# Nextomics/NextPolish2

Hardware: AMD Instinct MI355X
Metric: polished reference Mbp/s (whole node) at 30x HiFi + k21/k31; FASTA identical to oracle (higher is better)
Workload: dtype u8

## Files before the change

### nextpolish2_amd/csrc/np2_host.cpp

```cpp
#include "../../include/np2.h"
#include "np2_common.hpp"
#include "np2_kernels.hpp"
#include "np2_ctx.hpp"
#include "np2_phase_host.hpp"

#include <algorithm>
#include <atomic>
#include <thread>
#include <chrono>
#include <cstdio>
#include <cstdlib>
#include <cstring>
#include <map>
#include <mutex>
#include <stdexcept>
#include <string>
#include <unordered_map>
#include <unordered_set>
#include <future>
#include <functional>
#include <vector>

using namespace np2;

// ... 166 lines not shown
    std::vector<uint32_t> cur_lo(R), cur_up(R);
    for (uint32_t v = 0; v < R; ++v) {
        cur_lo[v] = vd.off_own[v], cur_up[v] = vd.off_own[v] + n_lo[v];
        vd.off_own[v + 1] = cur_up[v] + n_up[v];
    }
    vd.edges_own.resize(vd.off_own[R]);
    for (uint64_t i = 0; i < np; ++i) {
        uint32_t a, b;
        if (!listed(i, a, b)) continue;
        const int32_t same = (int32_t)(cn[i] & 0xFFFFu), neg = (int32_t)(cn[i] >> 16);
        const float w = (float)(neg >= 3 ? -neg : same - neg);
        vd.edges_own[cur_lo[b]++] = phase::Graph::Edge(a, w);
        vd.edges_own[cur_up[a]++] = phase::Graph::Edge(b, w);
    }
    vd.off = vd.off_own.data(), vd.edges = vd.edges_own.data(), vd.n_nokey = nokey;
    return true;
}

void vote_collect(np2_ctx *cx, np2_contig *c, PassCounts &pc, bool asref, bool use_all, int pass, uint32_t own_lo,
                  uint32_t own_hi, VoteData &vd, bool wide = false, uint64_t key_add = 0) {
    hipStream_t s = cx->stream;
    const uint32_t R = c->R, n_reg = pc.n_reg;
    RegionTables rt = region_tables(cx, n_reg);
    uint32_t NE = 0, NU = 0;
    vd = VoteData();
    vd.R = R;
    {
        EventTimer t(cx, "vote_phase");
        cx->reg_lable.ensure(n_reg + 2);
        cx->grp.ensure((size_t)pc.NC_cap + 2);
        cx->ecount.ensure(n_reg + 2);
        cx->eoff.ensure(std::max<size_t>(n_reg + 2, (size_t)c->L + 2));
        const size_t RP = ((size_t)R + 63) & ~(size_t)63;
        const size_t band_words = (size_t)R * EDGE_BAND;
        const size_t b_v = RP * 10, b_off = (((size_t)R + 2) * 4 + 15) & ~(size_t)15;
        uint8_t *vbuf;
        uint32_t *row_off;
        if (wide) {
            cx->votebuf.ensure(b_v);
            cx->band_off.ensure((size_t)R + 2);
            vbuf = cx->votebuf.p, row_off = cx->band_off.p;
        } else {
            cx->votepack.ensure(b_v + b_off + band_words * 2 * sizeof(phase::Graph::Edge) + 64);
            vbuf = cx->votepack.p, row_off = (uint32_t *)(cx->votepack.p + b_v);
        }
        uint32_t *v_first = (uint32_t *)vbuf;
        int32_t *v_refw = (int32_t *)(vbuf + RP * 4);
        uint8_t *v_seen = vbuf + RP * 8, *v_bad = vbuf + RP * 9;
        op_fill(cx, v_first, 0xFF, RP * 4);
        op_fill(cx, v_refw, 0, RP * 6);
        launch_vote_phase(s, rt, asref, use_all, cx->lq_start.p, own_lo, own_hi, cx->reg_lable.p, cx->grp.p, cx->ecount.p,
                          v_refw, v_seen, v_bad, v_first, cx->scal.p + S_ERR);
        exclusive_total_n(cx, cx->ecount.p, cx->eoff.p, n_reg);
        launch_vote_counts(s, v_first, v_bad, R, cx->scal.p + S_M1);
        cx->band.ensure(band_words + 4);
        cx->band_n.ensure((size_t)R + 2);
        op_fill(cx, cx->scal.p + S_M3, 0, 4);
        launch_edges_row(s, rt, cx->grp.p, cx->ecount.p, cx->pj.p, cx->pcount.p, cx->alive.p, R, cx->band.p, cx->band_n.p,
                         cx->scal.p + S_M3);
        if (wide) {
            exclusive_total_n(cx, cx->band_n.p, row_off, R);
            cx->ekey.ensure(band_words + 2);
            cx->eval.ensure(band_words + 2);
            launch_band_emit(s, cx->band.p, R, row_off, cx->ekey.p, cx->eval.p, cx->scal.p + S_NRAW, key_add);
        } else {
            cx->row_cnt.ensure((size_t)R + 2);
            launch_vote_rows_count(s, cx->band.p, cx->band_n.p, v_bad, use_all, R, cx->row_cnt.p, cx->scal.p + S_NOKEY);
            exclusive_total_n(cx, cx->row_cnt.p, row_off, R);
            launch_vote_rows_emit(s, cx->band.p, cx->band_n.p, v_bad, use_all, v_first, R, row_off, cx->votepack.p + b_v + b_off,
                                  cx->scal.p + S_NRAW, cx->scal.p + S_NOKEY);
        }
    }
    const size_t RP = ((size_t)R + 63) & ~(size_t)63;
    const size_t b_v = RP * 10, b_off = (((size_t)R + 2) * 4 + 15) & ~(size_t)15;
    auto per_read = [&](const uint8_t *vb) {
        vd.first_key.assign((const uint32_t *)vb, (const uint32_t *)vb + R);
        vd.ref_w.assign((const int32_t *)(vb + RP * 4), (const int32_t *)(vb + RP * 4) + R);
        vd.ref_seen.assign(vb + RP * 8, vb + RP * 8 + R);
        vd.bad.assign(vb + RP * 9, vb + RP * 9 + R);
    };
    bool far = false, have_per_read = false;
    {
        std::vector<uint32_t> sc;
        uint8_t *pin = nullptr;
        const size_t EB = sizeof(phase::Graph::Edge);
        static_assert(sizeof(phase::Graph::Edge) == 8 && alignof(phase::Graph::Edge) <= 8, "an edge is {u32 neighbour, f32 weight}");
        const uint32_t likely = (uint32_t)std::min<size_t>((size_t)R * EDGE_BAND * 2, std::max<size_t>((size_t)R * 128, 1u << 15));
        if (wide) {
            sc = fetch_scal(cx, cx->scal.p + S_M0, cx->eoff.p + n_reg);
        } else {
            pin = (uint8_t *)cx->pin_d2h.ensure(b_v + b_off + (size_t)likely * EB + 64);
            const uint32_t seq = ++cx->mbox_seq;
            launch_post(cx->stream, cx->scal.p, S_COUNT, cx->mbox_dev, seq, cx->scal.p + S_M0, cx->eoff.p + n_reg, nullptr, nullptr,
                        nullptr, nullptr, nullptr, nullptr, nullptr, nullptr);
            op_d2h(cx, pin, cx->votepack.p, b_v + b_off);
            launch_copy_counted(cx->stream, (uint32_t *)(pin + b_v + b_off), (const uint32_t *)(cx->votepack.p + b_v + b_off),
                                (const uint32_t *)(cx->votepack.p + b_v) + R, likely * (uint32_t)(EB / 4), (uint32_t)(EB / 4));
            op_sync(cx);
            if (__atomic_load_n(&cx->mbox_host[0], __ATOMIC_ACQUIRE) != seq)
                throw Np2Error(NP2_E_DEVICE, "mailbox not posted after a synchronisation");
            sc.assign(cx->mbox_host + 1, cx->mbox_host + 1 + S_COUNT);
        }
        check_region_err(cx, sc[S_ERR]);
        pc.resolve(sc);
        NE = sc[S_M0];
        if (!cx->trace && sc[S_M1] == 0 && sc[S_M2] == 0) {
            if (NE) throw Np2Error(NP2_E_DEVICE, "internal: pair edges without voting reads");
            return;
        }
        NU = sc[S_NRAW];
        far = sc[S_M3] != 0 || cx->hooks.edge_sort;
        if (!wide) cx->timing.host.push_back({far ? "vote_sort" : "vote_rows", 1.0f});
        if (!wide) {
            per_read(pin);
            have_per_read = true;
            vd.d_bad = cx->votepack.p + RP * 9;
            if (!far) {
                if (NU > likely) {
                    pin = (uint8_t *)cx->pin_d2h.ensure(b_v + b_off + (size_t)NU * EB + 64);
                    op_d2h(cx, pin, cx->votepack.p, b_v + b_off + (size_t)NU * EB);
// ... 2123 lines not shown
```

### nextpolish2_amd/csrc/np2_kernels.hpp

```cpp
#pragma once
#include <cstddef>
#include <cstdint>
#include <hip/hip_runtime.h>
#include "../../include/np2.h"
#include "np2_lookback.hpp"
#include "np2_launch.hpp"

namespace np2 {

static constexpr uint32_t TILE_SHIFT = 10;
static constexpr uint32_t TILE = 1u << TILE_SHIFT;
static constexpr uint32_t TILE_CAP = 4096;

static constexpr uint32_t DENSE_COLS = 4096;
struct ChunkDesc {
    uint64_t nib_off;
    uint64_t ckbase;
    uint32_t read, ts;
    uint32_t c0, ncols;
    uint32_t first_chunk;
    uint32_t aln_t_e, nck;
    uint32_t pad0;
    uint32_t pad[4];
};
// ... 208 lines not shown
static constexpr uint32_t PF_CAP_BIG = 3584;
static constexpr uint32_t PF_COV_MAX = 8192;
static constexpr uint32_t PF_REDO = 1u;
static constexpr uint32_t PF_NEED_BIG = 2u;
struct PfTile {
    const uint64_t *keys;
    const uint32_t *vals;
    const uint32_t *tile_n, *tile_scan;
    const uint16_t *pidx;
    const uint8_t *alive;
    const np2_read_t *reads;
    const uint32_t *tile_rd_off, *tile_rd;
    const uint8_t *refnib;
    uint16_t *slots;
    uint32_t *tile_cnt, *tile_lq;
    long long *tile_gain;
    uint32_t *flags, *n_bad, *bad_list, *n_bad2, *bad_list2;
    long long *end_rel;
    unsigned long long *gain_total;
    unsigned long long *prof;
    uint32_t L, n_tiles, bucket_cap;
    uint32_t cap_lim, cap_lim_big, halo_lim, cov_max;
    uint32_t big_enabled;
};
uint64_t pf_slot_entries(uint32_t n_tiles, uint64_t T);
void launch_pf_tile(hipStream_t s, const PfTile &a);
void launch_pf_compact(hipStream_t s, uint32_t n_tiles, const uint16_t *slots, const uint32_t *tile_scan, const uint32_t *tile_cnt,
                       const uint32_t *tile_coff, const uint32_t *tile_lqoff, uint32_t *cns_pos, uint8_t *cns_base,
                       uint8_t *cns_cls, uint8_t *lq_nothead, uint32_t *lq_list, uint32_t lq_cap, uint32_t *err, uint32_t *flags,
                       uint32_t *flags_out, uint32_t *n_bad, uint32_t *n_bad2);

struct RegionTables {
    const uint32_t *cand_off;
    const uint32_t *order;
    uint16_t *kscore;
    const uint32_t *seq_off;
    const uint8_t *seq;
    uint32_t n_reg;
};
struct RechPtrs {
    const void *groups;
    const uint32_t *job_off;
    const uint32_t *rech;
    const uint32_t *cand_off;
    const uint32_t *keep_list;
    const uint32_t *seq_off;
    const uint8_t *seq;
    const uint8_t *cns_base;
    uint32_t n_groups;
};
void launch_vote_phase(hipStream_t s, const RegionTables &rt, bool asref, bool use_all, const uint32_t *lq_start,
                       uint32_t own_lo, uint32_t own_hi, uint8_t *reg_lable, uint8_t *grp, uint32_t *ecount, int32_t *ref_w,
                       uint8_t *ref_seen, uint8_t *bad, uint32_t *first_reg, uint32_t *err);
void launch_vote_counts(hipStream_t s, const uint32_t *first_reg, const uint8_t *bad, uint32_t R, uint32_t *out);
void launch_edges_write(hipStream_t s, const RegionTables &rt, const uint8_t *reg_lable, const uint8_t *grp,
                        const uint32_t *ecount, const uint32_t *eoff, uint64_t *ekey, uint32_t *eval);
static constexpr uint32_t EDGE_BAND = 256;
void launch_edges_row(hipStream_t s, const RegionTables &rt, const uint8_t *grp, const uint32_t *ecount, const uint32_t *pj,
                      const uint32_t *pcount, const uint8_t *alive, uint32_t R, uint32_t *band, uint32_t *row_n, uint32_t *ovf);
void launch_band_emit(hipStream_t s, const uint32_t *band, uint32_t R, const uint32_t *row_off, uint64_t *ukey, uint32_t *uw,
                      uint32_t *n_out, uint64_t key_add = 0);
void launch_vote_rows_count(hipStream_t s, const uint32_t *band, const uint32_t *row_n, const uint8_t *bad, bool use_all, uint32_t R,
                            uint32_t *cnt, uint32_t *nokey);
void launch_vote_rows_emit(hipStream_t s, const uint32_t *band, const uint32_t *row_n, const uint8_t *bad, bool use_all,
                           const uint32_t *first_reg, uint32_t R, const uint32_t *off, void *edges, uint32_t *n_out, uint32_t *nokey);
void launch_edge_reduce(hipStream_t s, const uint64_t *ekey, const uint32_t *eval, uint32_t n, uint32_t *flag, uint32_t *wout);
void launch_edge_compact(hipStream_t s, const uint64_t *ekey, const uint32_t *flag, const uint32_t *idx, const uint32_t *wout,
                         uint32_t n, uint64_t *ukey, uint32_t *uw, uint32_t *n_out);
void launch_seed(hipStream_t s, const RegionTables &rt, int32_t max_indel_len, uint8_t *reg_lable, uint32_t *seed_cand,
                 uint32_t *keep_n, uint32_t *keep_list, uint16_t *keep_ks, uint32_t *err, uint32_t *rl_list = nullptr,
                 uint32_t *rl_cnt = nullptr, uint32_t rl_cap = 0);
uint32_t region_lb_blocks(uint32_t n_reg);
void launch_splice_find(hipStream_t s, const uint32_t *cns_pos, const uint32_t *M_p, const uint32_t *lq_start,
                        const uint32_t *lq_end, const uint8_t *reg_lable, uint8_t lable, uint32_t n_reg, uint32_t *idx_s,
                        uint32_t *idx_e, uint32_t *stuck);
void launch_splice_plan(hipStream_t s, const Lookback &lb, const uint8_t *reg_lable, uint8_t lable, uint32_t n_reg,
                        const uint32_t *stuck, const uint32_t *idx_s, const uint32_t *idx_e, const uint32_t *seed_cand,
                        const uint32_t *seq_off, uint32_t *ap_g, uint32_t *ap_s, uint32_t *ap_e, int32_t *ap_delta,
                        int32_t *ap_shift_incl, uint32_t *n_ap, const uint32_t *M_in, uint32_t *M_out, uint32_t out_cap , uint32_t *err);
void launch_splice_write(hipStream_t s, const uint32_t *in_pos, const uint8_t *in_base, const uint32_t *M_p, uint32_t M_cap,
                         const uint32_t *ap_g, const uint32_t *ap_s, const uint32_t *ap_e, const int32_t *ap_delta,
                         const int32_t *ap_shift_incl, const uint32_t *n_ap, uint32_t max_ap, const uint32_t *lq_start,
                         const uint32_t *seed_cand, const uint32_t *seq_off, const uint8_t *seq, uint32_t *out_pos,
                         uint8_t *out_base);
void launch_shard_bounds(hipStream_t s, const uint32_t *cns_pos, const uint32_t *M_p, const uint32_t *t, uint32_t *out);
void launch_rech_list(hipStream_t s, const Lookback &lb, const uint8_t *reg_lable, uint32_t n_reg, uint32_t *rech,
                      uint32_t *n_rech, unsigned long long *blob_bound, uint32_t *err);
void launch_rech_groups(hipStream_t s, const Lookback &lb, const uint32_t *rech, const uint32_t *n_rech_p, uint32_t max_rech,
                        const uint32_t *cns_pos, const uint32_t *M_p, const uint32_t *lq_start, const uint32_t *lq_end,
                        const uint32_t *keep_n, uint32_t ksize, const uint32_t *reg_maxlen, void *tmp_groups,
                        uint32_t *head_jobs, void *groups, uint32_t *job_off, uint32_t *n_groups, uint32_t *n_jobs,
                        unsigned long long *blob_bound, uint32_t *err);
size_t rech_group_bytes();
void launch_rech_job_len(hipStream_t s, const RechPtrs &p, uint32_t n_jobs, uint32_t *len);
void launch_rech_job_build(hipStream_t s, const RechPtrs &p, uint32_t n_jobs, const uint32_t *soff32, uint64_t *soff64,
                           uint8_t *blob);
void launch_rech_apply(hipStream_t s, const RechPtrs &p, const uint16_t *score, uint16_t *keep_ks);
void launch_rech_select(hipStream_t s, const uint32_t *rech, const uint32_t *n_rech_p, uint32_t max_rech,
                        const uint32_t *cand_off, const uint32_t *keep_n, const uint32_t *keep_list, const uint16_t *keep_ks,
                        const uint32_t *order, bool first_yak, uint8_t *reg_lable, uint32_t *seed_cand);
void launch_rech_relabel(hipStream_t s, uint8_t *reg_lable, uint32_t n_reg);
static constexpr uint32_t RL_CAP_LIST = 1024;
static constexpr uint32_t RL_CAP_JOBS = 2048;
static constexpr uint32_t RL_CAP_BLOB = 1u << 20;
static constexpr uint32_t RL_NREG_MAX = 400000;
enum : uint32_t { RL_N = 0, RL_NGROUPS, RL_NJOBS, RL_OFF, RL_STATE_WORDS };
struct RechList {
    const uint32_t *list_in;
    uint32_t *cnt_in;
    uint32_t *list_out, *cnt_out;
    uint32_t *st;
    uint32_t *rech;
    uint32_t *pos_lo, *pos_ub;
    void *groups, *tmp_groups;
    uint32_t *job_off, *blob_off, *glen;
    uint2 *job_ol;
// ... 43 lines not shown
```

### nextpolish2_amd/csrc/np2_regions.hip

```cpp
#include "np2_common.hpp"
#include "np2_kernels.hpp"
#include "np2_blockscan.hpp"
#include "np2_lookback.hpp"

namespace np2 {

static constexpr uint8_t LB_TEMP = 0x01, LB_SUCC = 0x80, LB_HETE = 0x40, LB_RECH = 0x20;

__device__ __forceinline__ uint32_t min_support(uint32_t n) { return n >= 9 ? 3u : (n >= 6 ? 2u : 1u); }

struct SubWave {
    uint32_t base;
    bool half;
    __device__ __forceinline__ uint64_t ballot(bool p) const {
        const uint64_t b = __ballot(p);
        return half ? (b >> base) & 0xFFFFFFFFull : b;
    }
    template <class T> __device__ __forceinline__ T shfl(T v, uint32_t j) const { return __shfl(v, (int)(base + j)); }
};

struct WaveStats {
    uint64_t eqmask;
    uint32_t stat;
    uint32_t c;
// ... 191 lines not shown
                    if (wgt < 0 && !use_all) bad[order] = 1;
                }
                const uint64_t V = ref_valid ? (valid & ~1ull) : valid;
                const uint32_t m = __builtin_popcountll(V);
                if (m >= 2 && owned) {
                    ne = m * (m - 1) / 2;
                    if ((V >> lane) & 1ull) atomicMin(&first_reg[order], g);
                }
            }
        }
        if (lane == 0) {
            reg_lable[g] = lable;
            ecount[g] = ne;
        }
    }
}

__device__ __forceinline__ void k_edges_write(const uint32_t np2_bid, const uint32_t np2_nb, RegionTables rt, const uint8_t *__restrict__ reg_lable,
                                                     const uint8_t *__restrict__ grp,
                                                     const uint32_t *__restrict__ ecount,
                                                     const uint32_t *__restrict__ eoff, uint64_t *__restrict__ ekey,
                                                     uint32_t *__restrict__ eval) {
    const uint32_t lane = threadIdx.x & 63;
    const uint32_t g = (uint32_t)__builtin_amdgcn_readfirstlane((int)((np2_bid * blockDim.x + threadIdx.x) >> 6));
    if (g >= rt.n_reg || ecount[g] == 0) return;
    const uint32_t c0 = rt.cand_off[g], n = rt.cand_off[g + 1] - c0;
    uint32_t order = 0xFFFFFFFFu, gi = 0;
    bool v = false;
    if (lane < n) {
        order = rt.order[c0 + lane];
        gi = grp[c0 + lane];
        v = rt.kscore[c0 + lane] > 0;
    }
    uint64_t V = __ballot(v);
    if ((V & 1ull) && __shfl(order, 0) == 0) V &= ~1ull;
    const bool mine = (V >> lane) & 1ull;
    const uint32_t cnt = mine ? __builtin_popcountll(lane == 63 ? 0ull : (V >> (lane + 1))) : 0u;
    uint32_t inc = cnt;
    for (int o = 1; o < 64; o <<= 1) {
        const uint32_t t = __shfl_up(inc, o);
        if (lane >= (uint32_t)o) inc += t;
    }
    uint32_t o = eoff[g] + inc - cnt;
    for (uint32_t j = 1; j < n; ++j) {
        const uint32_t oj = __shfl(order, j), gj = __shfl(gi, j);
        if (mine && j > lane && ((V >> j) & 1ull)) {
            ekey[o] = ((uint64_t)order << 32) | oj;
            eval[o] = (gj == gi) ? 1u : 0xFFFFFFFFu;
            ++o;
        }
    }
}

__device__ __forceinline__ void k_edges_row(const uint32_t np2_bid0, const uint32_t np2_nb, RegionTables rt, const uint8_t *__restrict__ grp,
                                            const uint32_t *__restrict__ ecount, const uint32_t *__restrict__ pj,
                                            const uint32_t *__restrict__ pcount, const uint8_t *__restrict__ alive, uint32_t R,
                                            uint32_t *__restrict__ band, uint32_t *__restrict__ row_n, uint32_t *__restrict__ ovf) {
    const uint32_t np2_bid = xcd_order(np2_bid0, np2_nb);
    __shared__ uint32_t s_row[4][EDGE_BAND];
    const uint32_t lane = threadIdx.x & 63, wv = (uint32_t)__builtin_amdgcn_readfirstlane((int)(threadIdx.x >> 6));
    const uint32_t a = np2_bid * 4 + wv;
    if (a >= R) return;
    uint32_t *row = s_row[wv];
    *reinterpret_cast<uint4 *>(row + lane * 4) = make_uint4(0, 0, 0, 0);
    uint32_t far = 0;
    const uint32_t n_span = (a != 0 && alive[a]) ? pcount[a] : 0u;
    const uint32_t j0 = n_span ? pj[a] : 0u;
    const uint32_t hl = lane & 31, hsel = lane >> 5;
    for (uint32_t base = 0; base < n_span; base += 64) {
        const uint32_t gl = j0 + base + lane;
        const bool in = base + lane < n_span && gl < rt.n_reg;
        const uint32_t c0l = in ? rt.cand_off[gl] : 0u, c1l = in ? rt.cand_off[gl + 1] : 0u;
        uint64_t het = __ballot(in && ecount[gl] != 0);
        while (het) {
            const uint32_t i0 = (uint32_t)__builtin_ctzll(het);
            het &= het - 1;
            const uint32_t c0a = (uint32_t)__builtin_amdgcn_readlane((int)c0l, (int)i0);
            const uint32_t na = (uint32_t)__builtin_amdgcn_readlane((int)c1l, (int)i0) - c0a;
            uint32_t c0b = 0, nb = 0;
            bool two = false;
            if (het && na <= 32) {
                const uint32_t i1 = (uint32_t)__builtin_ctzll(het);
                c0b = (uint32_t)__builtin_amdgcn_readlane((int)c0l, (int)i1);
                nb = (uint32_t)__builtin_amdgcn_readlane((int)c1l, (int)i1) - c0b;
                two = nb <= 32;
                if (two) het &= het - 1;
            }
            const uint32_t li = two ? hl : lane;
            const uint32_t c0 = (two && hsel) ? c0b : c0a, n = (two && hsel) ? nb : na;
            uint32_t order = 0xFFFFFFFFu, gi = 0;
            bool v = false;
            if (li < n) {
                order = rt.order[c0 + li];
                gi = grp[c0 + li];
                v = rt.kscore[c0 + li] > 0;
            }
            uint64_t V = __ballot(v);
            if ((V & 1ull) && __shfl(order, 0) == 0) V &= ~1ull;
            if (two && ((V >> 32) & 1ull) && __shfl(order, 32) == 0) V &= ~(1ull << 32);
            const uint64_t me = __ballot(order == a) & V;
            const uint64_t half_mask = two ? (hsel ? 0xFFFFFFFF00000000ull : 0x00000000FFFFFFFFull) : ~0ull;
            const uint64_t mine = me & half_mask;
            if (!me) continue;
            const uint32_t ga = __shfl(gi, mine ? (int)__builtin_ctzll(mine) : 0);
            if (mine && ((V >> lane) & 1ull) && order > a) {
                const uint32_t d = order - a - 1;
                if (d < EDGE_BAND)
                    atomicAdd(&row[d], gi == ga ? 1u : 0x10000u);
                else
                    ++far;
            }
        }
    }
    const uint4 w = *reinterpret_cast<const uint4 *>(row + lane * 4);
    uint32_t c = (w.x != 0) + (w.y != 0) + (w.z != 0) + (w.w != 0);
    for (int o = 32; o > 0; o >>= 1) c += __shfl_xor(c, o);
    if (c) *reinterpret_cast<uint4 *>(band + (uint64_t)a * EDGE_BAND + lane * 4) = w;
    if (lane == 0) row_n[a] = c;
    for (int o = 32; o > 0; o >>= 1) far += __shfl_xor(far, o);
    if (far && lane == 0) atomicAdd(ovf, far);
}
__device__ __forceinline__ void k_band_emit(const uint32_t np2_bid, const uint32_t np2_nb, const uint32_t *__restrict__ band, uint32_t R,
                                            const uint32_t *__restrict__ row_off, uint64_t *__restrict__ ukey,
                                            uint32_t *__restrict__ ucnt, uint32_t *__restrict__ n_out, uint64_t key_add) {
    const uint32_t lane = threadIdx.x & 63;
    const uint32_t a = (uint32_t)__builtin_amdgcn_readfirstlane((int)((np2_bid * blockDim.x + threadIdx.x) >> 6));
    if (a >= R) return;
    if (a == R - 1 && lane == 0) *n_out = row_off[R];
    if (row_off[a + 1] == row_off[a]) return;
    const uint4 w = *reinterpret_cast<const uint4 *>(band + (uint64_t)a * EDGE_BAND + lane * 4);
    const uint32_t v[4] = {w.x, w.y, w.z, w.w};
    const uint32_t c = (w.x != 0) + (w.y != 0) + (w.z != 0) + (w.w != 0);
    uint32_t inc = c;
    for (int o = 1; o < 64; o <<= 1) {
        const uint32_t t = __shfl_up(inc, o);
        if (lane >= (uint32_t)o) inc += t;
    }
    uint32_t o = row_off[a] + inc - c;
#pragma unroll
    for (uint32_t k = 0; k < 4; ++k)
        if (v[k]) {
            ukey[o] = (((uint64_t)a << 32) | (a + 1 + lane * 4 + k)) + key_add;
            ucnt[o] = v[k];
            ++o;
        }
}

__device__ __forceinline__ uint32_t vote_row_above(const uint32_t *__restrict__ band, const uint8_t *__restrict__ bad, uint32_t use_all,
                                                   uint32_t R, uint32_t v, uint32_t d) {
    const uint32_t b = v + 1 + d;
    if (b >= R) return 0;
    const uint32_t w = band[(uint64_t)v * EDGE_BAND + d];
    return (w != 0 && (use_all || !bad[b])) ? w : 0u;
}
__device__ __forceinline__ uint32_t vote_row_below(const uint32_t *__restrict__ band, const uint32_t *__restrict__ row_n,
                                                   const uint8_t *__restrict__ bad, uint32_t use_all, uint32_t v, int64_t a) {
    if (a < 1 || a >= (int64_t)v || v - (uint32_t)a > EDGE_BAND) return 0;
    if (row_n[a] == 0 || (!use_all && bad[a])) return 0;
    return band[(uint64_t)a * EDGE_BAND + (v - (uint32_t)a - 1)];
}
__device__ __forceinline__ float vote_weight(uint32_t w) {
    const int32_t same = (int32_t)(w & 0xFFFFu), neg = (int32_t)(w >> 16);
    return (float)(neg >= 3 ? -neg : same - neg);
}
__device__ __forceinline__ void k_vote_rows_count(const uint32_t np2_bid, const uint32_t np2_nb, const uint32_t *__restrict__ band,
                                                  const uint32_t *__restrict__ row_n, const uint8_t *__restrict__ bad, uint32_t use_all,
                                                  uint32_t R, uint32_t *__restrict__ cnt, uint32_t *__restrict__ nokey) {
    const uint32_t lane = threadIdx.x & 63;
    const uint32_t v = (uint32_t)__builtin_amdgcn_readfirstlane((int)((np2_bid * blockDim.x + threadIdx.x) >> 6));
    if (v >= R) return;
    if (v == 0 && lane == 0) *nokey = 0;
    uint32_t c = 0;
    if (v != 0 && (use_all || !bad[v])) {
        const bool own = row_n[v] != 0;
#pragma unroll
        for (uint32_t k = 0; k < EDGE_BAND / 64; ++k) {
            const uint32_t d = k * 64 + lane;
            if (own) c += vote_row_above(band, bad, use_all, R, v, d) != 0;
            c += vote_row_below(band, row_n, bad, use_all, v, (int64_t)v - 1 - d) != 0;
        }
    }
    for (int o = 32; o > 0; o >>= 1) c += __shfl_xor(c, o);
    if (lane == 0) cnt[v] = c;
}
__device__ __forceinline__ void k_vote_rows_emit(const uint32_t np2_bid, const uint32_t np2_nb, const uint32_t *__restrict__ band,
                                                 const uint32_t *__restrict__ row_n, const uint8_t *__restrict__ bad, uint32_t use_all,
                                                 const uint32_t *__restrict__ first_reg, uint32_t R, const uint32_t *__restrict__ off,
                                                 uint2 *__restrict__ edges, uint32_t *__restrict__ n_out, uint32_t *__restrict__ nokey) {
    const uint32_t lane = threadIdx.x & 63;
    const uint32_t v = (uint32_t)__builtin_amdgcn_readfirstlane((int)((np2_bid * blockDim.x + threadIdx.x) >> 6));
    if (v >= R) return;
    if (v == R - 1 && lane == 0) *n_out = off[R];
    if (v == 0) return;
    const bool own = row_n[v] != 0, live = use_all || !bad[v];
    const uint64_t lt = (1ull << lane) - 1;
    uint32_t o = off[v];
    const uint32_t end = off[v + 1];
    if (live && end != o) {
#pragma unroll
        for (uint32_t k = 0; k < EDGE_BAND / 64; ++k) {
            const int64_t a = (int64_t)v - EDGE_BAND + k * 64 + lane;
            const uint32_t w = vote_row_below(band, row_n, bad, use_all, v, a);
            const uint64_t m = __ballot(w != 0);
            const uint32_t at = o + (uint32_t)__popcll(m & lt);
            if (w != 0 && at < end) edges[at] = make_uint2((uint32_t)a, __float_as_uint(vote_weight(w)));
            o += (uint32_t)__popcll(m);
        }
    }
    if (!own) return;
    const bool v_key = first_reg[v] != 0xFFFFFFFFu;
    uint32_t nk = 0;
#pragma unroll
    for (uint32_t k = 0; k < EDGE_BAND / 64; ++k) {
        const uint32_t d = k * 64 + lane, b = v + 1 + d;
        if (b < R && band[(uint64_t)v * EDGE_BAND + d] != 0 && !(v_key && first_reg[b] != 0xFFFFFFFFu)) ++nk;
        const uint32_t w = live ? vote_row_above(band, bad, use_all, R, v, d) : 0u;
        const uint64_t m = __ballot(w != 0);
        const uint32_t at = o + (uint32_t)__popcll(m & lt);
        if (w != 0 && at < end) edges[at] = make_uint2(b, __float_as_uint(vote_weight(w)));
        o += (uint32_t)__popcll(m);
    }
    for (int x = 32; x > 0; x >>= 1) nk += __shfl_xor(nk, x);
    if (nk && lane == 0) atomicAdd(nokey, nk);
}

__device__ __forceinline__ void k_edge_reduce(const uint32_t np2_bid, const uint32_t np2_nb, const uint64_t *__restrict__ ekey, const uint32_t *__restrict__ eval, uint32_t n,
                              uint32_t *__restrict__ flag, uint32_t *__restrict__ wout) {
    uint32_t i = np2_bid * blockDim.x + threadIdx.x;
    if (i >= n) return;
    const uint64_t k = ekey[i];
    if (i > 0 && ekey[i - 1] == k) {
        flag[i] = 0;
        return;
    }
    int32_t sum = 0, neg = 0;
    for (uint32_t j = i; j < n && ekey[j] == k; ++j) {
// ... 801 lines not shown
    }
    __syncthreads();
    const uint32_t stuck = s_stuck;
    uint32_t flag[RL_ITEMS], fsum = 0;
    int32_t delta[RL_ITEMS], dsum_t = 0;
#pragma unroll
    for (uint32_t k = 0; k < RL_ITEMS; ++k) {
        flag[k] = (tid * RL_ITEMS + k < n && g[k] + 1 > stuck) ? 1u : 0u;
        delta[k] = 0;
        if (flag[k]) {
            const uint32_t c = seed_cand[g[k]];
            delta[k] = (int32_t)(seq_off[c + 1] - seq_off[c]) - (int32_t)(e[k] - s[k]);
        }
        fsum += flag[k], dsum_t += delta[k];
    }
    uint32_t cnt, dsum;
    uint32_t lo = block_excl_scan<OpAdd, 4>(fsum, sh, cnt);
    uint32_t ld = block_excl_scan<OpAdd, 4>((uint32_t)dsum_t, sh, dsum);
#pragma unroll
    for (uint32_t k = 0; k < RL_ITEMS; ++k) {
        if (flag[k]) {
            ap_g[lo] = g[k];
            ap_s[lo] = s[k];
            ap_e[lo] = e[k];
            ap_delta[lo] = delta[k];
            ap_shift_incl[lo] = (int32_t)ld + delta[k];
        }
        lo += flag[k];
        ld += (uint32_t)delta[k];
    }
    if (tid == 0) splice_plan_total(M, dsum, cnt, out_cap, n_ap, M_out, err);
    uint32_t keep[RL_ITEMS], ksum = 0;
#pragma unroll
    for (uint32_t k = 0; k < RL_ITEMS; ++k) {
        keep[k] = 0;
        if (tid * RL_ITEMS + k < n) {
            const uint8_t l = rech_relabel(reg_lable[g[k]]);
            reg_lable[g[k]] = l;
            keep[k] = (l & LB_RECH) ? 1u : 0u;
        }
        ksum += keep[k];
    }
    uint32_t n_keep;
    uint32_t lk = block_excl_scan<OpAdd, 4>(ksum, sh, n_keep);
#pragma unroll
    for (uint32_t k = 0; k < RL_ITEMS; ++k) {
        if (keep[k]) a.list_out[lk] = g[k];
        lk += keep[k];
    }
    if (tid == 0) *a.cnt_in = 0, *a.cnt_out = last_round ? 0u : n_keep;
}

__device__ __forceinline__ void k_vote_counts(const uint32_t np2_bid, const uint32_t np2_nb, const uint32_t *__restrict__ first_reg, const uint8_t *__restrict__ bad,
                                                      uint32_t R, uint32_t *__restrict__ out) {
    __shared__ uint32_t sk[16], sb[16];
    uint32_t nk = 0, nb = 0;
    for (uint32_t r = threadIdx.x; r < R; r += 1024) {
        nk += first_reg[r] != 0xFFFFFFFFu ? 1u : 0u;
        nb += bad[r] ? 1u : 0u;
    }
    for (int o = 32; o > 0; o >>= 1) {
        nk += __shfl_xor(nk, o);
        nb += __shfl_xor(nb, o);
    }
    if ((threadIdx.x & 63) == 0) {
        sk[threadIdx.x >> 6] = nk;
        sb[threadIdx.x >> 6] = nb;
    }
    __syncthreads();
    if (threadIdx.x == 0) {
        uint32_t a = 0, b = 0;
        for (int i = 0; i < 16; ++i) {
            a += sk[i];
            b += sb[i];
        }
        out[0] = a;
        out[1] = b;
    }
}

static inline dim3 g1(uint64_t n, uint32_t bs = 256) { return dim3((unsigned)((n + bs - 1) / bs)); }

void launch_vote_phase(hipStream_t s, const RegionTables &rt, bool asref, bool use_all, const uint32_t *lq_start,
                       uint32_t own_lo, uint32_t own_hi, uint8_t *reg_lable, uint8_t *grp, uint32_t *ecount, int32_t *ref_w,
                       uint8_t *ref_seen, uint8_t *bad, uint32_t *first_reg, uint32_t *err) {
    if (rt.n_reg)
        NP2_LAUNCH(k_vote_phase, g1((uint64_t)((rt.n_reg + 1) / 2) * 64), 256, s, rt, asref ? 1u : 0u, use_all ? 1u : 0u, lq_start, own_lo, own_hi, reg_lable, grp, ecount, ref_w, ref_seen, bad, first_reg, err);
}
void launch_vote_counts(hipStream_t s, const uint32_t *first_reg, const uint8_t *bad, uint32_t R, uint32_t *out) {
    NP2_LAUNCH(k_vote_counts, dim3(1), 1024, s, first_reg, bad, R, out);
}
void launch_edges_write(hipStream_t s, const RegionTables &rt, const uint8_t *reg_lable, const uint8_t *grp,
                        const uint32_t *ecount, const uint32_t *eoff, uint64_t *ekey, uint32_t *eval) {
    if (rt.n_reg)
        NP2_LAUNCH(k_edges_write, g1((uint64_t)rt.n_reg * 64), 256, s, rt, reg_lable, grp, ecount, eoff, ekey, eval);
}
void launch_edges_row(hipStream_t s, const RegionTables &rt, const uint8_t *grp, const uint32_t *ecount, const uint32_t *pj,
                      const uint32_t *pcount, const uint8_t *alive, uint32_t R, uint32_t *band, uint32_t *row_n, uint32_t *ovf) {
    if (R) NP2_LAUNCH(k_edges_row, g1((uint64_t)R * 64), 256, s, rt, grp, ecount, pj, pcount, alive, R, band, row_n, ovf);
}
void launch_vote_rows_count(hipStream_t s, const uint32_t *band, const uint32_t *row_n, const uint8_t *bad, bool use_all, uint32_t R,
                            uint32_t *cnt, uint32_t *nokey) {
    if (R) NP2_LAUNCH(k_vote_rows_count, g1((uint64_t)R * 64), 256, s, band, row_n, bad, use_all ? 1u : 0u, R, cnt, nokey);
}
void launch_vote_rows_emit(hipStream_t s, const uint32_t *band, const uint32_t *row_n, const uint8_t *bad, bool use_all,
                           const uint32_t *first_reg, uint32_t R, const uint32_t *off, void *edges, uint32_t *n_out, uint32_t *nokey) {
    if (R) NP2_LAUNCH(k_vote_rows_emit, g1((uint64_t)R * 64), 256, s, band, row_n, bad, use_all ? 1u : 0u, first_reg, R, off, (uint2 *)edges, n_out, nokey);
}
void launch_band_emit(hipStream_t s, const uint32_t *band, uint32_t R, const uint32_t *row_off, uint64_t *ukey, uint32_t *uw,
                      uint32_t *n_out, uint64_t key_add) {
    if (R) NP2_LAUNCH(k_band_emit, g1((uint64_t)R * 64), 256, s, band, R, row_off, ukey, uw, n_out, key_add);
}
void launch_edge_reduce(hipStream_t s, const uint64_t *ekey, const uint32_t *eval, uint32_t n, uint32_t *flag,
                        uint32_t *wout) {
    if (n) NP2_LAUNCH(k_edge_reduce, g1(n), 256, s, ekey, eval, n, flag, wout);
}
void launch_edge_compact(hipStream_t s, const uint64_t *ekey, const uint32_t *flag, const uint32_t *idx,
                         const uint32_t *wout, uint32_t n, uint64_t *ukey, uint32_t *uw, uint32_t *n_out) {
    if (n) NP2_LAUNCH(k_edge_compact, g1(n), 256, s, ekey, flag, idx, wout, n, ukey, uw, n_out);
}
void launch_seed(hipStream_t s, const RegionTables &rt, int32_t max_indel_len, uint8_t *reg_lable, uint32_t *seed_cand,
                 uint32_t *keep_n, uint32_t *keep_list, uint16_t *keep_ks, uint32_t *err, uint32_t *rl_list, uint32_t *rl_cnt,
                 uint32_t rl_cap) {
    if (rt.n_reg)
        NP2_LAUNCH(k_seed, g1((uint64_t)((rt.n_reg + 1) / 2) * 64), 256, s, rt, max_indel_len, reg_lable, seed_cand, keep_n, keep_list, keep_ks, err, rl_list, rl_cnt, rl_cap);
}
uint32_t region_lb_blocks(uint32_t n_reg) { return (n_reg + 256 * LB_REG_ITEMS - 1) / (256 * LB_REG_ITEMS); }
void launch_splice_find(hipStream_t s, const uint32_t *cns_pos, const uint32_t *M_p, const uint32_t *lq_start,
                        const uint32_t *lq_end, const uint8_t *reg_lable, uint8_t lable, uint32_t n_reg,
                        uint32_t *idx_s, uint32_t *idx_e, uint32_t *stuck) {
    NP2_LAUNCH(k_splice_find, g1(n_reg), 256, s, cns_pos, M_p, lq_start, lq_end, reg_lable, lable, n_reg, idx_s, idx_e, stuck);
}
void launch_splice_plan(hipStream_t s, const Lookback &lb, const uint8_t *reg_lable, uint8_t lable, uint32_t n_reg,
                        const uint32_t *stuck, const uint32_t *idx_s, const uint32_t *idx_e, const uint32_t *seed_cand,
                        const uint32_t *seq_off, uint32_t *ap_g, uint32_t *ap_s, uint32_t *ap_e, int32_t *ap_delta,
                        int32_t *ap_shift_incl, uint32_t *n_ap, const uint32_t *M_in, uint32_t *M_out, uint32_t out_cap, uint32_t *err) {
    const uint32_t nb = region_lb_blocks(n_reg);
    NP2_LAUNCH(k_splice_plan, dim3(nb), 256, s, lb, nb, reg_lable, lable, n_reg, stuck, idx_s, idx_e, seed_cand, seq_off, ap_g, ap_s, ap_e, ap_delta, ap_shift_incl, n_ap, M_in, M_out, out_cap, err);
}
void launch_splice_write(hipStream_t s, const uint32_t *in_pos, const uint8_t *in_base, const uint32_t *M_p, uint32_t M_cap,
                         const uint32_t *ap_g, const uint32_t *ap_s, const uint32_t *ap_e, const int32_t *ap_delta,
                         const int32_t *ap_shift_incl, const uint32_t *n_ap, uint32_t max_ap, const uint32_t *lq_start,
                         const uint32_t *seed_cand, const uint32_t *seq_off, const uint8_t *seq, uint32_t *out_pos,
                         uint8_t *out_base) {
    NP2_LAUNCH(k_splice_bases, dim3((M_cap + SPLICE_SPAN - 1) / SPLICE_SPAN), 256, s, in_pos, in_base, M_p, ap_s, ap_e, ap_shift_incl, n_ap, out_pos, out_base);
    if (max_ap)
        NP2_LAUNCH(k_splice_seeds, g1((uint64_t)max_ap * 8, 256), 256, s, ap_g, ap_s, ap_delta, ap_shift_incl, n_ap, lq_start, seed_cand, seq_off, seq, out_pos, out_base);
}
void launch_shard_bounds(hipStream_t s, const uint32_t *cns_pos, const uint32_t *M_p, const uint32_t *t, uint32_t *out) {
    NP2_LAUNCH(k_shard_bounds, dim3(1), 64, s, cns_pos, M_p, t[0], t[1], t[2], t[3], t[4], t[5], out);
}
void launch_rech_list(hipStream_t s, const Lookback &lb, const uint8_t *reg_lable, uint32_t n_reg, uint32_t *rech,
                      uint32_t *n_rech, unsigned long long *blob_bound, uint32_t *err) {
    const uint32_t nb = region_lb_blocks(n_reg);
    NP2_LAUNCH(k_rech_list, dim3(nb), 256, s, lb, nb, reg_lable, n_reg, rech, n_rech, blob_bound, err);
}
// ... 53 lines not shown
```

Baseline: 4500.

## Fuse vote row counting into edge row kernel and unroll candidate walk

Removes the separate vote_rows_count kernel: the edge-row kernel now counts per-row edges with atomics on both endpoints while it still holds the band row in registers. The overflow and nokey zeroing moves into vote_counts, which also clears the cnt array, dropping a fill op. The candidate walk is unrolled four ways to batch loads, and the row popcount uses ballots. This saves launches and a band re-read, but adds global atomics on cnt and changes how the count is derived, which risks output divergence.

```diff
diff --git a/nextpolish2_amd/csrc/np2_host.cpp b/nextpolish2_amd/csrc/np2_host.cpp
--- a/nextpolish2_amd/csrc/np2_host.cpp
+++ b/nextpolish2_amd/csrc/np2_host.cpp
@@ -242,20 +242,19 @@
         launch_vote_phase(s, rt, asref, use_all, cx->lq_start.p, own_lo, own_hi, cx->reg_lable.p, cx->grp.p, cx->ecount.p,
                           v_refw, v_seen, v_bad, v_first, cx->scal.p + S_ERR);
         exclusive_total_n(cx, cx->ecount.p, cx->eoff.p, n_reg);
-        launch_vote_counts(s, v_first, v_bad, R, cx->scal.p + S_M1);
+        if (!wide) cx->row_cnt.ensure((size_t)R + 2);
+        launch_vote_counts(s, v_first, v_bad, R, cx->scal.p + S_M1, cx->scal.p + S_M3, wide ? nullptr : cx->row_cnt.p,
+                           wide ? nullptr : cx->scal.p + S_NOKEY);
         cx->band.ensure(band_words + 4);
         cx->band_n.ensure((size_t)R + 2);
-        op_fill(cx, cx->scal.p + S_M3, 0, 4);
         launch_edges_row(s, rt, cx->grp.p, cx->ecount.p, cx->pj.p, cx->pcount.p, cx->alive.p, R, cx->band.p, cx->band_n.p,
-                         cx->scal.p + S_M3);
+                         cx->scal.p + S_M3, v_bad, use_all, wide ? nullptr : cx->row_cnt.p);
         if (wide) {
             exclusive_total_n(cx, cx->band_n.p, row_off, R);
             cx->ekey.ensure(band_words + 2);
             cx->eval.ensure(band_words + 2);
             launch_band_emit(s, cx->band.p, R, row_off, cx->ekey.p, cx->eval.p, cx->scal.p + S_NRAW, key_add);
         } else {
-            cx->row_cnt.ensure((size_t)R + 2);
-            launch_vote_rows_count(s, cx->band.p, cx->band_n.p, v_bad, use_all, R, cx->row_cnt.p, cx->scal.p + S_NOKEY);
             exclusive_total_n(cx, cx->row_cnt.p, row_off, R);
             launch_vote_rows_emit(s, cx->band.p, cx->band_n.p, v_bad, use_all, v_first, R, row_off, cx->votepack.p + b_v + b_off,
                                   cx->scal.p + S_NRAW, cx->scal.p + S_NOKEY);
diff --git a/nextpolish2_amd/csrc/np2_kernels.hpp b/nextpolish2_amd/csrc/np2_kernels.hpp
--- a/nextpolish2_amd/csrc/np2_kernels.hpp
+++ b/nextpolish2_amd/csrc/np2_kernels.hpp
@@ -284,16 +284,16 @@
 void launch_vote_phase(hipStream_t s, const RegionTables &rt, bool asref, bool use_all, const uint32_t *lq_start,
                        uint32_t own_lo, uint32_t own_hi, uint8_t *reg_lable, uint8_t *grp, uint32_t *ecount, int32_t *ref_w,
                        uint8_t *ref_seen, uint8_t *bad, uint32_t *first_reg, uint32_t *err);
-void launch_vote_counts(hipStream_t s, const uint32_t *first_reg, const uint8_t *bad, uint32_t R, uint32_t *out);
+void launch_vote_counts(hipStream_t s, const uint32_t *first_reg, const uint8_t *bad, uint32_t R, uint32_t *out, uint32_t *ovf,
+                        uint32_t *cnt, uint32_t *nokey);
 void launch_edges_write(hipStream_t s, const RegionTables &rt, const uint8_t *reg_lable, const uint8_t *grp,
                         const uint32_t *ecount, const uint32_t *eoff, uint64_t *ekey, uint32_t *eval);
 static constexpr uint32_t EDGE_BAND = 256;
 void launch_edges_row(hipStream_t s, const RegionTables &rt, const uint8_t *grp, const uint32_t *ecount, const uint32_t *pj,
-                      const uint32_t *pcount, const uint8_t *alive, uint32_t R, uint32_t *band, uint32_t *row_n, uint32_t *ovf);
+                      const uint32_t *pcount, const uint8_t *alive, uint32_t R, uint32_t *band, uint32_t *row_n, uint32_t *ovf,
+                      const uint8_t *bad, bool use_all, uint32_t *cnt);
 void launch_band_emit(hipStream_t s, const uint32_t *band, uint32_t R, const uint32_t *row_off, uint64_t *ukey, uint32_t *uw,
                       uint32_t *n_out, uint64_t key_add = 0);
-void launch_vote_rows_count(hipStream_t s, const uint32_t *band, const uint32_t *row_n, const uint8_t *bad, bool use_all, uint32_t R,
-                            uint32_t *cnt, uint32_t *nokey);
 void launch_vote_rows_emit(hipStream_t s, const uint32_t *band, const uint32_t *row_n, const uint8_t *bad, bool use_all,
                            const uint32_t *first_reg, uint32_t R, const uint32_t *off, void *edges, uint32_t *n_out, uint32_t *nokey);
 void launch_edge_reduce(hipStream_t s, const uint64_t *ekey, const uint32_t *eval, uint32_t n, uint32_t *flag, uint32_t *wout);
diff --git a/nextpolish2_amd/csrc/np2_regions.hip b/nextpolish2_amd/csrc/np2_regions.hip
--- a/nextpolish2_amd/csrc/np2_regions.hip
+++ b/nextpolish2_amd/csrc/np2_regions.hip
@@ -267,10 +267,13 @@
     }
 }
 
+static constexpr int EDGE_WALK_U = 4;
 __device__ __forceinline__ void k_edges_row(const uint32_t np2_bid0, const uint32_t np2_nb, RegionTables rt, const uint8_t *__restrict__ grp,
                                             const uint32_t *__restrict__ ecount, const uint32_t *__restrict__ pj,
                                             const uint32_t *__restrict__ pcount, const uint8_t *__restrict__ alive, uint32_t R,
-                                            uint32_t *__restrict__ band, uint32_t *__restrict__ row_n, uint32_t *__restrict__ ovf) {
+                                            uint32_t *__restrict__ band, uint32_t *__restrict__ row_n, uint32_t *__restrict__ ovf,
+                                            const uint8_t *__restrict__ bad, uint32_t use_all, uint32_t *__restrict__ cnt) {
+    constexpr int U = EDGE_WALK_U;
     const uint32_t np2_bid = xcd_order(np2_bid0, np2_nb);
     __shared__ uint32_t s_row[4][EDGE_BAND];
     const uint32_t lane = threadIdx.x & 63, wv = (uint32_t)__builtin_amdgcn_readfirstlane((int)(threadIdx.x >> 6));
@@ -288,52 +291,83 @@
         const uint32_t c0l = in ? rt.cand_off[gl] : 0u, c1l = in ? rt.cand_off[gl + 1] : 0u;
         uint64_t het = __ballot(in && ecount[gl] != 0);
         while (het) {
-            const uint32_t i0 = (uint32_t)__builtin_ctzll(het);
-            het &= het - 1;
-            const uint32_t c0a = (uint32_t)__builtin_amdgcn_readlane((int)c0l, (int)i0);
-            const uint32_t na = (uint32_t)__builtin_amdgcn_readlane((int)c1l, (int)i0) - c0a;
-            uint32_t c0b = 0, nb = 0;
-            bool two = false;
-            if (het && na <= 32) {
-                const uint32_t i1 = (uint32_t)__builtin_ctzll(het);
-                c0b = (uint32_t)__builtin_amdgcn_readlane((int)c0l, (int)i1);
-                nb = (uint32_t)__builtin_amdgcn_readlane((int)c1l, (int)i1) - c0b;
-                two = nb <= 32;
-                if (two) het &= het - 1;
-            }
-            const uint32_t li = two ? hl : lane;
-            const uint32_t c0 = (two && hsel) ? c0b : c0a, n = (two && hsel) ? nb : na;
-            uint32_t order = 0xFFFFFFFFu, gi = 0;
-            bool v = false;
-            if (li < n) {
-                order = rt.order[c0 + li];
-                gi = grp[c0 + li];
-                v = rt.kscore[c0 + li] > 0;
-            }
-            uint64_t V = __ballot(v);
-            if ((V & 1ull) && __shfl(order, 0) == 0) V &= ~1ull;
-            if (two && ((V >> 32) & 1ull) && __shfl(order, 32) == 0) V &= ~(1ull << 32);
-            const uint64_t me = __ballot(order == a) & V;
-            const uint64_t half_mask = two ? (hsel ? 0xFFFFFFFF00000000ull : 0x00000000FFFFFFFFull) : ~0ull;
-            const uint64_t mine = me & half_mask;
-            if (!me) continue;
-            const uint32_t ga = __shfl(gi, mine ? (int)__builtin_ctzll(mine) : 0);
-            if (mine && ((V >> lane) & 1ull) && order > a) {
-                const uint32_t d = order - a - 1;
-                if (d < EDGE_BAND)
-                    atomicAdd(&row[d], gi == ga ? 1u : 0x10000u);
-                else
-                    ++far;
+            bool two[U];
+            uint32_t c0[U], n[U];
+#pragma unroll
+            for (int u = 0; u < U; ++u) {
+                const bool on = het != 0;
+                const uint32_t i0 = on ? (uint32_t)__builtin_ctzll(het) : 0u;
+                het &= het - 1;
+                const uint32_t c0a = (uint32_t)__builtin_amdgcn_readlane((int)c0l, (int)i0);
+                const uint32_t na = on ? (uint32_t)__builtin_amdgcn_readlane((int)c1l, (int)i0) - c0a : 0u;
+                uint32_t c0b = 0, nb = 0;
+                two[u] = false;
+                if (het && na <= 32) {
+                    const uint32_t i1 = (uint32_t)__builtin_ctzll(het);
+                    c0b = (uint32_t)__builtin_amdgcn_readlane((int)c0l, (int)i1);
+                    nb = (uint32_t)__builtin_amdgcn_readlane((int)c1l, (int)i1) - c0b;
+                    two[u] = nb <= 32;
+                    if (two[u]) het &= het - 1;
+                }
+                c0[u] = ((two[u] && hsel) ? c0b : c0a) + (two[u] ? hl : lane);
+                n[u] = (two[u] && hsel) ? nb : na;
+            }
+            uint32_t order[U], gi[U], ks[U];
+#pragma unroll
+            for (int u = 0; u < U; ++u) {
+                order[u] = 0xFFFFFFFFu, gi[u] = 0, ks[u] = 0;
+                if ((two[u] ? hl : lane) < n[u]) {
+                    order[u] = rt.order[c0[u]];
+                    gi[u] = grp[c0[u]];
+                    ks[u] = rt.kscore[c0[u]];
+                }
+            }
+#pragma unroll
+            for (int u = 0; u < U; ++u) {
+                const bool v = ks[u] > 0;
+                const uint64_t me = __ballot(v && order[u] == a);
+                if (me) {
+                    constexpr uint32_t NO_GRP = 0x100;
+                    const uint64_t me_lo = two[u] ? (me & 0xFFFFFFFFull) : me, me_hi = two[u] ? (me >> 32 << 32) : me;
+                    const uint32_t ga_lo = me_lo ? (uint32_t)__builtin_amdgcn_readlane((int)gi[u], (int)__builtin_ctzll(me_lo)) : NO_GRP;
+                    const uint32_t ga_hi = me_hi ? (uint32_t)__builtin_amdgcn_readlane((int)gi[u], (int)__builtin_ctzll(me_hi)) : NO_GRP;
+                    const uint32_t ga = hsel ? ga_hi : ga_lo;
+                    if (v && order[u] > a && ga != NO_GRP) {
+                        const uint32_t d = order[u] - a - 1;
+                        if (d < EDGE_BAND)
+                            atomicAdd(&row[d], gi[u] == ga ? 1u : 0x10000u);
+                        else
+                            ++far;
+                    }
+                }
             }
         }
     }
     const uint4 w = *reinterpret_cast<const uint4 *>(row + lane * 4);
-    uint32_t c = (w.x != 0) + (w.y != 0) + (w.z != 0) + (w.w != 0);
-    for (int o = 32; o > 0; o >>= 1) c += __shfl_xor(c, o);
+    const uint32_t c = (uint32_t)(__popcll(__ballot(w.x != 0)) + __popcll(__ballot(w.y != 0)) + __popcll(__ballot(w.z != 0)) +
+                                  __popcll(__ballot(w.w != 0)));
     if (c) *reinterpret_cast<uint4 *>(band + (uint64_t)a * EDGE_BAND + lane * 4) = w;
     if (lane == 0) row_n[a] = c;
-    for (int o = 32; o > 0; o >>= 1) far += __shfl_xor(far, o);
-    if (far && lane == 0) atomicAdd(ovf, far);
+    if (__ballot(far != 0)) {
+        for (int o = 32; o > 0; o >>= 1) far += __shfl_xor(far, o);
+        if (lane == 0) atomicAdd(ovf, far);
+    }
+    if (cnt && c && (use_all || !bad[a])) {
+        const uint32_t wk[4] = {w.x, w.y, w.z, w.w};
+        uint32_t e = 0, fl[4] = {0, 0, 0, 0};
+        if (!use_all) {
+#pragma unroll
+            for (uint32_t k = 0; k < 4; ++k) fl[k] = bad[min(a + 1 + lane * 4 + k, R - 1)];
+        }
+#pragma unroll
+        for (uint32_t k = 0; k < 4; ++k) {
+            const uint32_t b = a + 1 + lane * 4 + k;
+            const bool edge = wk[k] != 0 && b < R && !fl[k];
+            if (edge) atomicAdd(&cnt[b], 1u);
+            e += (uint32_t)__popcll(__ballot(edge));
+        }
+        if (e && lane == 0) atomicAdd(&cnt[a], e);
+    }
 }
 __device__ __forceinline__ void k_band_emit(const uint32_t np2_bid, const uint32_t np2_nb, const uint32_t *__restrict__ band, uint32_t R,
                                             const uint32_t *__restrict__ row_off, uint64_t *__restrict__ ukey,
@@ -377,26 +411,6 @@
 __device__ __forceinline__ float vote_weight(uint32_t w) {
     const int32_t same = (int32_t)(w & 0xFFFFu), neg = (int32_t)(w >> 16);
     return (float)(neg >= 3 ? -neg : same - neg);
-}
-__device__ __forceinline__ void k_vote_rows_count(const uint32_t np2_bid, const uint32_t np2_nb, const uint32_t *__restrict__ band,
-                                                  const uint32_t *__restrict__ row_n, const uint8_t *__restrict__ bad, uint32_t use_all,
-                                                  uint32_t R, uint32_t *__restrict__ cnt, uint32_t *__restrict__ nokey) {
-    const uint32_t lane = threadIdx.x & 63;
-    const uint32_t v = (uint32_t)__builtin_amdgcn_readfirstlane((int)((np2_bid * blockDim.x + threadIdx.x) >> 6));
-    if (v >= R) return;
-    if (v == 0 && lane == 0) *nokey = 0;
-    uint32_t c = 0;
-    if (v != 0 && (use_all || !bad[v])) {
-        const bool own = row_n[v] != 0;
-#pragma unroll
-        for (uint32_t k = 0; k < EDGE_BAND / 64; ++k) {
-            const uint32_t d = k * 64 + lane;
-            if (own) c += vote_row_above(band, bad, use_all, R, v, d) != 0;
-            c += vote_row_below(band, row_n, bad, use_all, v, (int64_t)v - 1 - d) != 0;
-        }
-    }
-    for (int o = 32; o > 0; o >>= 1) c += __shfl_xor(c, o);
-    if (lane == 0) cnt[v] = c;
 }
 __device__ __forceinline__ void k_vote_rows_emit(const uint32_t np2_bid, const uint32_t np2_nb, const uint32_t *__restrict__ band,
                                                  const uint32_t *__restrict__ row_n, const uint8_t *__restrict__ bad, uint32_t use_all,
@@ -1304,12 +1318,18 @@
 }
 
 __device__ __forceinline__ void k_vote_counts(const uint32_t np2_bid, const uint32_t np2_nb, const uint32_t *__restrict__ first_reg, const uint8_t *__restrict__ bad,
-                                                      uint32_t R, uint32_t *__restrict__ out) {
+                                                      uint32_t R, uint32_t *__restrict__ out, uint32_t *__restrict__ ovf,
+                                                      uint32_t *__restrict__ cnt, uint32_t *__restrict__ nokey) {
     __shared__ uint32_t sk[16], sb[16];
     uint32_t nk = 0, nb = 0;
+    if (threadIdx.x == 0) {
+        *ovf = 0;
+        if (nokey) *nokey = 0;
+    }
     for (uint32_t r = threadIdx.x; r < R; r += 1024) {
         nk += first_reg[r] != 0xFFFFFFFFu ? 1u : 0u;
         nb += bad[r] ? 1u : 0u;
+        if (cnt) cnt[r] = 0;
     }
     for (int o = 32; o > 0; o >>= 1) {
         nk += __shfl_xor(nk, o);
@@ -1339,8 +1359,9 @@
     if (rt.n_reg)
         NP2_LAUNCH(k_vote_phase, g1((uint64_t)((rt.n_reg + 1) / 2) * 64), 256, s, rt, asref ? 1u : 0u, use_all ? 1u : 0u, lq_start, own_lo, own_hi, reg_lable, grp, ecount, ref_w, ref_seen, bad, first_reg, err);
 }
-void launch_vote_counts(hipStream_t s, const uint32_t *first_reg, const uint8_t *bad, uint32_t R, uint32_t *out) {
-    NP2_LAUNCH(k_vote_counts, dim3(1), 1024, s, first_reg, bad, R, out);
+void launch_vote_counts(hipStream_t s, const uint32_t *first_reg, const uint8_t *bad, uint32_t R, uint32_t *out, uint32_t *ovf,
+                        uint32_t *cnt, uint32_t *nokey) {
+    NP2_LAUNCH(k_vote_counts, dim3(1), 1024, s, first_reg, bad, R, out, ovf, cnt, nokey);
 }
 void launch_edges_write(hipStream_t s, const RegionTables &rt, const uint8_t *reg_lable, const uint8_t *grp,
                         const uint32_t *ecount, const uint32_t *eoff, uint64_t *ekey, uint32_t *eval) {
@@ -1348,12 +1369,10 @@
         NP2_LAUNCH(k_edges_write, g1((uint64_t)rt.n_reg * 64), 256, s, rt, reg_lable, grp, ecount, eoff, ekey, eval);
 }
 void launch_edges_row(hipStream_t s, const RegionTables &rt, const uint8_t *grp, const uint32_t *ecount, const uint32_t *pj,
-                      const uint32_t *pcount, const uint8_t *alive, uint32_t R, uint32_t *band, uint32_t *row_n, uint32_t *ovf) {
-    if (R) NP2_LAUNCH(k_edges_row, g1((uint64_t)R * 64), 256, s, rt, grp, ecount, pj, pcount, alive, R, band, row_n, ovf);
-}
-void launch_vote_rows_count(hipStream_t s, const uint32_t *band, const uint32_t *row_n, const uint8_t *bad, bool use_all, uint32_t R,
-                            uint32_t *cnt, uint32_t *nokey) {
-    if (R) NP2_LAUNCH(k_vote_rows_count, g1((uint64_t)R * 64), 256, s, band, row_n, bad, use_all ? 1u : 0u, R, cnt, nokey);
+                      const uint32_t *pcount, const uint8_t *alive, uint32_t R, uint32_t *band, uint32_t *row_n, uint32_t *ovf,
+                      const uint8_t *bad, bool use_all, uint32_t *cnt) {
+    static_assert(Sig<decltype(&k_edges_row)>::N >= 17, "a one-group batch of the default line is 17 contigs");
+    if (R) NP2_LAUNCH(k_edges_row, g1((uint64_t)R * 64), 256, s, rt, grp, ecount, pj, pcount, alive, R, band, row_n, ovf, bad, use_all ? 1u : 0u, cnt);
 }
 void launch_vote_rows_emit(hipStream_t s, const uint32_t *band, const uint32_t *row_n, const uint8_t *bad, bool use_all,
                            const uint32_t *first_reg, uint32_t R, const uint32_t *off, void *edges, uint32_t *n_out, uint32_t *nokey) {
```

Result: no change. 4511 (median of 2 runs) (+0.2%).
